# ZJU-Robotics-Lab/GEM

Hardware: AMD Instinct MI355X
Metric: fused points/sec into 600x600 grid; achieved HBM GB/s vs roofline (higher is better)
Workload: dtype f32

## Files before the change

gem_amd/build.py:

```python
from __future__ import annotations

import os
import shutil
import subprocess
from pathlib import Path

ROOT = Path(__file__).resolve().parent
CSRC = ROOT / "csrc"
LIBDIR = ROOT / "lib"
LIB = LIBDIR / "libgem_hip.so"

SOURCES = [CSRC / "gem_kernels.hip", CSRC / "gem_frame_lean.hip", CSRC / "gem_sort.hip", CSRC / "gem_capi.cpp", CSRC / "gem_capi_core.cpp", CSRC / "gem_capi_pipeline.cpp", CSRC / "gem_capi_comm.cpp",
           CSRC / "gem_clean.hip", CSRC / "gem_capi_clean.cpp", CSRC / "gem_local.hip", CSRC / "gem_capi_local.cpp",
           CSRC / "gem_voxel.hip", CSRC / "gem_capi_voxel.cpp", CSRC / "gem_global.hip", CSRC / "gem_capi_global.cpp",
           CSRC / "gem_compose.hip", CSRC / "gem_capi_compose.cpp", CSRC / "gem_costmap.hip", CSRC / "gem_capi_costmap.cpp",
           CSRC / "gem_octree.hip", CSRC / "gem_capi_octree.cpp", CSRC / "gem_depth.hip", CSRC / "gem_capi_depth.cpp",
           CSRC / "gem_history.hip", CSRC / "gem_capi_history.cpp",
           CSRC / "gem_footprint.hip", CSRC / "gem_capi_footprint.cpp", CSRC / "gem_inflate.hip", CSRC / "gem_capi_inflate.cpp",
           CSRC / "gem_mapgrid.hip", CSRC / "gem_capi_mapgrid.cpp", CSRC / "gem_critics.hip", CSRC / "gem_capi_critics.cpp",
           CSRC / "gem_trajgen.hip", CSRC / "gem_capi_trajgen.cpp", CSRC / "gem_navplan.hip", CSRC / "gem_capi_navplan.cpp",
           CSRC / "gem_frontier.hip", CSRC / "gem_capi_frontier.cpp", CSRC / "gem_obstacle.hip", CSRC / "gem_capi_obstacle.cpp",
           CSRC / "gem_voxlayer.hip", CSRC / "gem_capi_voxlayer.cpp"]
HEADERS = [CSRC / "gem_device.hpp", CSRC / "gem_kernels.hpp", CSRC / "gem_frame_lean.hpp", CSRC / "gem_frame_tile.hpp", CSRC / "gem_frame_sort.hpp", CSRC / "gem_wave.hpp", CSRC / "gem_compact.hpp", CSRC / "gem_transport.hpp", CSRC / "gem_hostcopy.hpp", CSRC / "gem_capi_internal.hpp", CSRC / "gem_plan.hpp", CSRC / "gem_clean.hpp", CSRC / "gem_local.hpp", CSRC / "gem_voxel.hpp", CSRC / "gem_global.hpp", CSRC / "gem_compose.hpp", CSRC / "gem_costmap.hpp", CSRC / "gem_lsd.hpp", CSRC / "gem_octree.hpp", CSRC / "gem_depth.hpp", CSRC / "gem_history.hpp", CSRC / "gem_footprint.hpp", CSRC / "gem_inflate.hpp", CSRC / "gem_mapgrid.hpp", CSRC / "gem_score_device.hpp", CSRC / "gem_critics.hpp", CSRC / "gem_trajgen.hpp", CSRC / "gem_sincos.hpp",
           CSRC / "gem_navplan.hpp", CSRC / "gem_navpath.hpp", CSRC / "gem_frontier.hpp", CSRC / "gem_costmap_host.hpp", CSRC / "gem_rounds.hpp", CSRC / "gem_tile_round.hpp", CSRC / "gem_obstacle.hpp", CSRC / "gem_voxlayer.hpp", ROOT.parent / "include" / "gem_hip_voxlayer.h", ROOT.parent / "include" / "gem_hip_frontier.h", ROOT.parent / "include" / "gem_hip_obstacle.h",
           ROOT.parent / "include" / "gem_hip_debug.h", ROOT.parent / "include" / "gem_hip.h", ROOT.parent / "include" / "gem_hip_history.h",
           ROOT.parent / "include" / "gem_hip_footprint.h", ROOT.parent / "include" / "gem_hip_inflate.h", ROOT.parent / "include" / "gem_hip_mapgrid.h",
           ROOT.parent / "include" / "gem_hip_critics.h", ROOT.parent / "include" / "gem_hip_trajgen.h", ROOT.parent / "include" / "gem_hip_navplan.h"]

FLAGS = [
    "--offload-arch=gfx950", "-O3", *(["-g"] if os.environ.get("GEM_DEBUG_BUILD") else []), "-std=c++17", "-ffp-contract=off", "-fPIC", "-shared",
    "-Wno-unused-value", "-Wno-unused-result",
    *os.environ.get("GEM_BUILD_DEFINES", "").split(),
]

SOURCE_FLAGS = {
    "gem_frame_lean.hip": ["-mllvm", "-amdgpu-kernarg-preload-count=14"],
}

# ... 99 lines not shown
```

gem_amd/csrc/gem_capi.cpp:

```cpp
#include "gem_capi_internal.hpp"
#include "gem_clean.hpp"
#include "gem_costmap.hpp"

namespace gemi {

int ensure_ray(gem_handle* h)
{
    if (h->ray.p) return GEM_OK;
    const int rc = ensure(h, h->ray, ((size_t)h->cells * 2 + 4) * sizeof(uint32_t));
    if (rc) return rc;
    GEM_HIP(h, hipMemsetAsync(static_cast<uint32_t*>(h->ray.p) + h->cells, 0, 4 * sizeof(uint32_t), h->stream));
    return GEM_OK;
}

static int queue_increment(gem_handle* h, float var_update)
{
    if (!(var_update >= 0.f)) h->floor_dirty = true;
    if (h->n_pending == kMaxPending) { int rc = flush_pending(h, false); if (rc) return rc; }
    h->pending[h->n_pending++] = var_update;
    return GEM_OK;
}

static int run_batch(gem_handle* h, int n_sweeps, const gem_frame_params* params, const float4* xyzi, const long long* offsets, const float* var_updates, bool caller_device)
{
// ... 186 lines not shown
    for (auto& ep : h->pool) { hipEventDestroy(ep.a); hipEventDestroy(ep.b); }
    local_free(h);
    global_free(h);
    costmap_free(h);
    history_free(h);
    octree_free(h);
    if (h->layers.elevation) hipFree(h->layers.elevation);
    if (h->d_counters) hipFree(h->d_counters);
    for (Arena* a : {&h->stage, &h->scratch, &h->dbg, &h->color, &h->ray, &h->sh_dev, &h->sh_recv_hv[0], &h->sh_recv_key[0], &h->sh_recv_rng[0],
                     &h->sh_recv_hv[1], &h->sh_recv_key[1], &h->sh_recv_rng[1], &h->sh_ranges, &h->published[0], &h->published[1],
                     &h->clean_cnt, &h->vox_state, &h->vox_hist, &h->vox_rec, &h->vox_tmp, &h->vox_out[0], &h->vox_out[1]}) if (a->p) hipFree(a->p);
    if (h->sh_host) hipHostFree(h->sh_host);
    if (h->form_seen) hipHostFree(h->form_seen);
    for (auto& b : h->pb) {
        for (Arena* a : {&b.rec, &b.srt, &b.seg, &b.flag, &b.gflag, &b.tables, &b.s_hv1, &b.s_hv2, &b.s_key1, &b.s_key2, &b.s_src1, &b.s_src2,
                         &b.s_cnt1, &b.s_cnt2, &b.s_misc, &b.s_ranges, &b.s_shard, &b.s_blkcnt}) if (a->p) hipFree(a->p);
        if (b.host_tables) hipHostFree(b.host_tables);
        if (b.tables_done) hipEventDestroy(b.tables_done);
        if (b.bin_done) hipEventDestroy(b.bin_done);
        if (b.fuse_done) hipEventDestroy(b.fuse_done);
    }
    if (h->copy_done) hipEventDestroy(h->copy_done);
    if (h->hstage) hipHostFree(h->hstage);
    for (auto& ev : h->ev_stage) if (ev) hipEventDestroy(ev);
    if (h->stage_read) hipEventDestroy(h->stage_read);
    for (auto& ev : h->ev_half) if (ev) hipEventDestroy(ev);
    if (h->switch_done) hipEventDestroy(h->switch_done);
    release_streams(h->device, h->streams);
    delete h;
}

// ... 4 lines not shown
    hipSetDevice(h->device);
    { const int rcd = settle(h); if (rcd) return rcd; }
    GEM_HIP(h, hipStreamSynchronize(h->stream));
    if (h->bin_stream) GEM_HIP(h, hipStreamSynchronize(h->bin_stream));
    if (h->bin_stream2) GEM_HIP(h, hipStreamSynchronize(h->bin_stream2));
    h->stream = hip_stream ? static_cast<hipStream_t>(hip_stream) : h->own_stream;
    return GEM_OK;
}

int gem_wait_event(gem_handle* h, void* hip_event)
{
    if (!h || !hip_event) return GEM_ERR_INVALID;
    std::lock_guard<std::mutex> lk(h->mu);
    hipSetDevice(h->device);
    hipEvent_t ev = static_cast<hipEvent_t>(hip_event);
    GEM_HIP(h, hipStreamWaitEvent(h->stream, ev, 0));
    if (h->bin_stream) GEM_HIP(h, hipStreamWaitEvent(h->bin_stream, ev, 0));
    if (h->bin_stream2) GEM_HIP(h, hipStreamWaitEvent(h->bin_stream2, ev, 0));
    h->main_reads_pb = true;
    return GEM_OK;
}

int gem_synchronize(gem_handle* h)
{
    ApiRange api_range(h, "gem_synchronize");
    if (!h) return GEM_ERR_INVALID;
    std::lock_guard<std::mutex> lk(h->mu);
    hipSetDevice(h->device);
    { const int rcd = settle(h); if (rcd) return rcd; }
    GEM_HIP(h, hipStreamSynchronize(h->stream));
// ... 237 lines not shown
    if (!h || n_sweeps <= 0 || !params || !offsets) return h ? fail(h, GEM_ERR_INVALID, "gem_add_batch_device: bad argument") : GEM_ERR_INVALID;
    std::lock_guard<std::mutex> lk(h->mu);
    hipSetDevice(h->device);
    { const int rcs = shard_finish_locked(h); if (rcs) return rcs; }
    for (int s = 0; s < n_sweeps; ++s) if (offsets[s + 1] < offsets[s]) return fail(h, GEM_ERR_INVALID, "gem_add_batch_device: offsets not monotone");
    return run_batch(h, n_sweeps, params, static_cast<const float4*>(d_xyzi), offsets, var_updates, true);
}

int gem_mapvar_update(gem_handle* h, float var_update)
{
    ApiRange api_range(h, "gem_mapvar_update");
    if (!h) return GEM_ERR_INVALID;
    std::lock_guard<std::mutex> lk(h->mu);
    hipSetDevice(h->device);
    { const int rcs = shard_finish_locked(h); if (rcs) return rcs; }
    return queue_increment(h, var_update);
}

static void* layer_ptr(gem_handle* h, int layer)
{
    switch (layer) {
    case GEM_LAYER_ELEVATION: return h->layers.elevation;
    case GEM_LAYER_VARIANCE:  return h->layers.variance;
    case GEM_LAYER_INTENSITY: return h->layers.intensity;
    case GEM_LAYER_TRAVER:    return h->layers.traver;
    case GEM_LAYER_LOWEST:    return h->layers.lowest;
    case GEM_LAYER_COLOR_R:   return h->layers.colorR;
    case GEM_LAYER_COLOR_G:   return h->layers.colorG;
    case GEM_LAYER_COLOR_B:   return h->layers.colorB;
    case GEM_LAYER_ROUGH:     return h->layers.rough;
// ... 248 lines not shown
    if (h->row0 != 0 || h->row1 != h->L) return fail(h, GEM_ERR_INVALID, "gem_raytracing: not available on a row-strip handle");
    int rc = flush_pending(h, false);
    if (rc) return rc;
    if ((rc = ensure_ray(h))) return rc;
    uint32_t* list = static_cast<uint32_t*>(h->ray.p);
    GEM_HIP(h, launch_raytracing(h->stream, h->layers, h->L, h->start[0], h->start[1], h->sensor_z, h->cfg.obstacle_threshold,
                                 h->row0, h->row1, list, list + h->cells, (int)(h->ray_calls++ & 1u), reinterpret_cast<float*>(list + h->cells + 4), h->ray_depth, h->ray_lanes));
    return GEM_OK;
}

int gem_set_timing(gem_handle* h, int enabled)
{
    if (!h) return GEM_ERR_INVALID;
    std::lock_guard<std::mutex> lk(h->mu);
    hipSetDevice(h->device);
    { const int rcd = settle(h); if (rcd) return rcd; }
    h->timing = enabled != 0;
    h->step_timed = h->timing && h->tp_x != nullptr && h->nranks > 1;
    return GEM_OK;
}

int gem_set_counting(gem_handle* h, int enabled)
{
    if (!h) return GEM_ERR_INVALID;
    std::lock_guard<std::mutex> lk(h->mu);
    hipSetDevice(h->device);
    { const int rcd = settle(h); if (rcd) return rcd; }
    h->counting = enabled != 0;
    return GEM_OK;
}

// ... 19 lines not shown
int gem_debug_set(gem_handle* h, const char* key, long long value)
{
    if (!h || !key) return GEM_ERR_INVALID;
    std::lock_guard<std::mutex> lk(h->mu);
    hipSetDevice(h->device);
    { const int rcd = settle(h); if (rcd) return rcd; }
    const std::string k(key);
    if (k == "fuse_variant")            { if (value < 10 || value > 12) return fail(h, GEM_ERR_INVALID, "fuse_variant: 10..12"); h->fuse_variant = (int)value; }
    else if (k == "tile_shift")         { if (value != 0 && value != 4 && value != 5) return fail(h, GEM_ERR_INVALID, "tile_shift: 0, 4 or 5"); h->ts = (int)value; }
    else if (k == "defer")              h->defer = value != 0;
    else if (k == "walk_always_wait")   h->walk_always_wait = value != 0;
    else if (k == "defer_walk")         { const int rcw = flush_walk(h); if (rcw) return rcw; h->defer_walk = value != 0; }
    else if (k == "dense_min")          { if (value < 0 || value > 0xffffffffll) return fail(h, GEM_ERR_INVALID, "dense_min: 0 .. 2^32 - 1"); h->dense_min = (unsigned)value; }
    else if (k == "dbg_sweep")          h->dbg_sweep = (int)value;
    else if (k == "dbg_frame")          h->dbg_frame = value != 0;
    else if (k == "frame_lean")         { if (value < 0 || value > 2) return fail(h, GEM_ERR_INVALID, "frame_lean: 0 (generic), 1 (lean) or 2 (the host picks)"); h->frame_lean = (int)value; }
    else if (k == "overlap")            h->overlap = value != 0;
    else if (k == "overlap_min_points") { if (value < 0) return fail(h, GEM_ERR_INVALID, "overlap_min_points: >= 0"); h->overlap_min_points = value; h->sort_overlap_min_points = value; }
    else if (k == "sort_path")          h->sort_path = value != 0;
    else if (k == "sort_min_points")    { if (value < 0) return fail(h, GEM_ERR_INVALID, "sort_min_points: >= 0"); h->sort_min_points = value; h->sort_min_points_batch = value; }
    else if (k == "walk_permute")       h->walk_permute = value != 0;
    else if (k == "trace")              h->trace = value != 0;
    else if (k == "stream_roles") {
        if (h->stream != h->own_stream) return fail(h, GEM_ERR_INVALID, "stream_roles: caller-provided stream in use");
        for (hipStream_t st : {h->own_stream, h->bin_stream, h->bin_stream2, h->tab_stream}) hipStreamSynchronize(st);
        const hipStream_t cur[4] = {h->own_stream, h->bin_stream, h->bin_stream2, h->tab_stream};
        const int d[4] = {(int)(value / 1000 % 10), (int)(value / 100 % 10), (int)(value / 10 % 10), (int)(value % 10)};
        bool seen[4] = {false, false, false, false};
        for (int i = 0; i < 4; ++i) { if (d[i] < 0 || d[i] > 3 || seen[d[i]]) return fail(h, GEM_ERR_INVALID, "stream_roles: not a permutation of 0123"); seen[d[i]] = true; }
        h->own_stream = cur[d[0]]; h->bin_stream = cur[d[1]]; h->bin_stream2 = cur[d[2]]; h->tab_stream = cur[d[3]];
// ... 36 lines not shown
    const std::string k(key);
    if (k == "arena_allocations") *out = h->arena_allocations;
    else if (k == "hstage_allocations") *out = h->hstage_allocations;
    else if (k == "copy_threads") *out = h->copy_threads;
    else if (k == "xfer_upload_memcpy_ns") *out = h->xfer_ns[0];
    else if (k == "xfer_upload_enqueue_ns") *out = h->xfer_ns[1];
    else if (k == "xfer_download_enqueue_ns") *out = h->xfer_ns[2];
    else if (k == "xfer_download_wait_ns") *out = h->xfer_ns[3];
    else if (k == "xfer_download_memcpy_ns") *out = h->xfer_ns[4];
    else if (k == "sort_fallbacks") *out = h->sort_fallbacks;
    else if (k == "compose_far_points") *out = h->compose.far_points;
    else if (k == "compose_sum_ns") *out = h->compose.sum_ns;
    else if (k == "walks_unwaited") *out = h->walks_unwaited;
    else if (k == "frame_lean_launches") *out = h->frame_lean_launches;
    else if (k == "frame_generic_launches") *out = h->frame_generic_launches;
    else if (k == "frame_form_seen") *out = h->form_seen ? (long long)*static_cast<volatile const uint32_t*>(h->form_seen) : 0;
    else if (k == "walks_left") *out = h->walks_left;
    else if (k == "history_cull") *out = h->history_cull ? 1 : 0;
    else if (k == "obstacle_direct") *out = h->obstacle_direct ? 1 : 0;
    else if (k == "nav_chunk") *out = h->nav_chunk;
    else if (k == "front_chunk") *out = h->front_chunk;
    else if (k == "history_blocks") *out = h->history.enabled ? cost_mark_blocks(h->history.len) : 0;
    else if (k == "history_blocks_culled") { hipSetDevice(h->device); return history_blocks_culled(h, out); }
    else if (k == "step_pending") *out = h->step.valid ? 1 : 0;
    else if (k == "step_exchange_bytes_out") *out = h->xbytes_out;
    else if (k == "step_exchange_bytes_in") *out = h->xbytes_in;
    else if (k == "gather_bytes_out") *out = h->gbytes_out;
    else if (k == "gather_bytes_in") *out = h->gbytes_in;
    else if (k.rfind("step_", 0) == 0) {
        int a = -1, b = -1;
// ... 44 lines not shown
```

gem_amd/csrc/gem_capi_core.cpp:

```cpp
#include "gem_capi_internal.hpp"

#include <cfloat>
#include <dlfcn.h>

namespace gemi {

thread_local std::string g_create_error;

namespace {
typedef int (*roctx_push_fn)(const char*);
typedef int (*roctx_pop_fn)();
std::once_flag g_roctx_once;
roctx_push_fn g_roctx_push = nullptr;
roctx_pop_fn g_roctx_pop = nullptr;
}

bool roctx_load()
{
    std::call_once(g_roctx_once, [] {
        for (const char* lib : {"librocprofiler-sdk-roctx.so", "librocprofiler-sdk-roctx.so.1", "libroctx64.so", "libroctx64.so.4"}) {
            void* so = dlopen(lib, RTLD_NOW | RTLD_GLOBAL);
            if (!so) continue;
            g_roctx_push = reinterpret_cast<roctx_push_fn>(dlsym(so, "roctxRangePushA"));
            g_roctx_pop = reinterpret_cast<roctx_pop_fn>(dlsym(so, "roctxRangePop"));
// ... 300 lines not shown
{
    hipEvent_t e = nullptr;
    hipEventCreate(&e);
    (void)h;
    return e;
}

void fold_events(gem_handle* h)
{
    for (auto& ep : h->events) {
        float ms = 0.f;
        if (hipEventSynchronize(ep.b) == hipSuccess && hipEventElapsedTime(&ms, ep.a, ep.b) == hipSuccess) {
            if (ep.kind == 0)      { h->stats.ms_bin += ms; h->stats.launches_bin++; }
            else if (ep.kind == 1) { h->stats.ms_fuse += ms; h->stats.launches_fuse++; }
            else if (ep.kind == 2) { h->stats.ms_frame += ms; h->stats.launches_frame++; }
            else if (ep.kind == 9) { h->stats.ms_walk += ms; h->stats.launches_walk++; }
            else                   { h->stats.ms_sort[ep.kind - 3] += ms; if (ep.kind == 3) h->stats.launches_sort++; }
        }
        else (void)hipGetLastError();
        h->pool.push_back(ep);
    }
    h->events.clear();
}

bool frame_launch_lean(gem_handle* h, bool fused_lean, bool bin_fast)
{
    const bool seen = h->form_seen && *static_cast<volatile const uint32_t*>(h->form_seen) != 0u;
    const bool lean = fused_lean && bin_fast && (h->frame_lean == 1 || (h->frame_lean == 2 && !seen));
    ++(lean ? h->frame_lean_launches : h->frame_generic_launches);
    return lean;
}

int flush_deferred(gem_handle* h)
{
    if (!h->deferred.valid) return GEM_OK;
    h->deferred.valid = false;
    h->main_reads_pb = true;
    if (h->dbg_frame) h->deferred.fa.dbg = nullptr;
    Timed t(h, 1);
    gem::BinArgs no_bin{};
    const bool lean = frame_launch_lean(h, h->deferred.lean_binned, true);
    GEM_HIP(h, launch_frame(h->stream, h->deferred.fa, no_bin, h->deferred.attr, lean, t.events()));
    return GEM_OK;
}

int flush_walk(gem_handle* h)
{
    if (!h->dwalk.valid) return GEM_OK;
    h->dwalk.valid = false;
    gem_handle::PassBuffers& pb = h->pb[h->dwalk.slot];
    if (!h->walk_always_wait && hipEventQuery(pb.bin_done) == hipSuccess) ++h->walks_unwaited;
    else { (void)hipGetLastError(); GEM_HIP(h, hipStreamWaitEvent(h->stream, pb.bin_done, 0)); }
    {
        Timed t(h, 9);
        GEM_HIP(h, h->dwalk.block_form ? launch_block_walk(h->stream, h->dwalk.wa, h->dwalk.attr, t.events()) : launch_walk(h->stream, h->dwalk.wa, h->dwalk.attr, t.events()));
    }
    GEM_HIP(h, hipEventRecord(pb.fuse_done, h->stream)); pb.fuse_recorded = true;
// ... 96 lines not shown
```

gem_amd/csrc/gem_capi_internal.hpp:

```cpp
#pragma once

#include "../../include/gem_hip.h"
#include "../../include/gem_hip_debug.h"
#include "gem_kernels.hpp"
#include "gem_plan.hpp"
#include "gem_hostcopy.hpp"
#include "gem_transport.hpp"

#include <hip/hip_runtime.h>
#include <rccl/rccl.h>

#include <chrono>
#include <cmath>
#include <cstdio>
#include <cstdlib>
#include <cstring>
#include <memory>
#include <mutex>
#include <string>
#include <vector>

using namespace gem;

namespace gem { struct CriticsArgs; struct FootSpec; struct CostGeom; }
// ... 45 lines not shown
        size_t host_cap = 0;
        hipEvent_t tables_done = nullptr;
        bool tables_recorded = false;
        std::vector<unsigned char> tab_key;
        int tab_src = 0;
        hipStream_t tab_upload_stream = nullptr;
        hipEvent_t bin_done = nullptr, fuse_done = nullptr;
        bool fuse_recorded = false;
        uint32_t epoch = 0;
    } pb[4];
    unsigned pass = 0, sort_pass = 0;
    uint32_t sort_epoch = 0;
    int sort_streams = 2;
    bool trace = false;
    int sort_ring = 3;
    struct Deferred { bool valid = false; FuseArgs fa{}; int ts = 0, attr = 0; bool lean_binned = false; } deferred;
    uint32_t* form_seen = nullptr;
    int  frame_lean = 2;
    long long frame_lean_launches = 0, frame_generic_launches = 0;
    struct DeferredWalk { bool valid = false; WalkArgs wa{}; bool block_form = false; int attr = 0; unsigned slot = 0; } dwalk;
    bool defer_walk = true;
    long long xbytes_out = 0, xbytes_in = 0, gbytes_out = 0, gbytes_in = 0;
    bool roctx = false;
    bool walk_always_wait = false;
    long long walks_unwaited = 0, walks_left = 0;
    bool defer = true;
    hipStream_t bin_stream = nullptr;
    hipStream_t bin_stream2 = nullptr;
    hipStream_t tab_stream = nullptr;
    hipEvent_t switch_done = nullptr;
    bool main_reads_pb = false;
// ... 279 lines not shown
    gem_handle* h; EventPair ep{};
    bool on;
    Timed(gem_handle* hh, int kind) : h(hh), on(hh->timing && kind >= 0)
    {
        if (!on) return;
        if (!h->pool.empty()) { ep = h->pool.back(); h->pool.pop_back(); }
        else { ep.a = get_event(h); ep.b = get_event(h); }
        ep.kind = kind;
    }
    LaunchEvents events() const { LaunchEvents e; if (on) { e.start = ep.a; e.stop = ep.b; } return e; }
    ~Timed() { if (on) h->events.push_back(ep); }
};

void fold_events(gem_handle* h);
int flush_deferred(gem_handle* h);
bool frame_launch_lean(gem_handle* h, bool fused_lean, bool bin_fast);
int flush_walk(gem_handle* h);
int flush_local(gem_handle* h);
int wait_gather(gem_handle* h);
void local_free(gem_handle* h);
int local_grid_count(gem_handle* h, uint32_t* n);
int local_export_to(gem_handle* h, void* dst, uint32_t n_grid, bool clear);
void compose_free(gem_handle* h);
int compose_check(gem_handle* h, const gem_compose_params* p, const char* what);
int compose_split(gem_handle* h, const gem_compose_params* p, bool want_road, bool want_obstacle, uint32_t tot[3], double* out_threshold);
void octree_free(gem_handle* h);
void global_free(gem_handle* h);
void history_free(gem_handle* h);
int history_check_room(gem_handle* h, long long n, const char* what);
int history_reserve(gem_handle* h, long long extra);
int history_append_device(gem_handle* h, const void* d_src, long long n);
// ... 94 lines not shown
```

gem_amd/csrc/gem_capi_pipeline.cpp:

```cpp
#include "gem_capi_internal.hpp"
#include "gem_clean.hpp"

namespace gemi {

static bool sort_bins_fit(int bins) { return sort_shape(bins, true, kSortChunkRecords).lds <= 160 * 1024; }
PlanEnv plan_env(const gem_handle* h)
{
    PlanEnv e{};
    e.L = h->L; e.ts = h->ts; e.sort_form = h->sort_form; e.sort_passes = h->sort_passes; e.sort_chunk = h->sort_chunk; e.sort_ring = h->sort_ring;
    e.sort_path = h->sort_path; e.track_lowest = h->track_lowest; e.sort_min_points = h->sort_min_points; e.sort_min_points_batch = h->sort_min_points_batch;
    return e;
}
SortGeometry sort_geometry(const gem_handle* h, int n_sweeps, bool block_form) { return sort_digits(h->L, h->sort_passes, n_sweeps, block_form, sort_bins_fit); }

static int stage_batch_tables(gem_handle* h, gem_handle::PassBuffers& pb, const TablesPlan& t, unsigned char** host = nullptr)
{
    if (t.total > pb.tables.cap) pb.tab_key.clear();
    const int rc = ensure(h, pb.tables, t.total);
    if (rc) return rc;
    if (t.total > pb.host_cap) {
        if (pb.tables_recorded) GEM_HIP(h, hipEventSynchronize(pb.tables_done));
        if (pb.host_tables) GEM_HIP(h, hipHostFree(pb.host_tables));
        pb.host_tables = nullptr; pb.host_cap = 0;
        GEM_HIP(h, hipHostMalloc(&pb.host_tables, t.total * 2, hipHostMallocDefault));
// ... 313 lines not shown
    std::vector<long long> cut_offsets;
    std::vector<int> orig0;
    if (plan.n_sweeps != in.n_sweeps) {
        const int ns = plan.n_sweeps;
        if (in.src == 0) cut_params.assign(ns, *in.params);
        cut_offsets.resize(ns + 1); orig0.resize(ns);
        for (int s = 0; s <= ns; ++s) cut_offsets[s] = std::min<long long>(in.n, (long long)s * kSweepPoints);
        for (int s = 0; s < ns; ++s) orig0[s] = (int)cut_offsets[s];
        in.n_sweeps = ns; in.params = in.src == 0 ? cut_params.data() : nullptr; in.offsets = cut_offsets.data(); in.var_updates = nullptr; in.sweep_orig0 = orig0.data();
    }
    const bool batched = in.n_sweeps > 1;
    const int U = kUnit, B = plan.B, bpad = plan.bpad;
    const bool dense = h->n_pending > 0 || h->floor_dirty || (batched && in.var_updates != nullptr);

    if (B == 0) {
        if (batched && in.var_updates)
            for (int s = 0; s < in.n_sweeps; ++s) {
                if (h->n_pending == kMaxPending) { int rc = flush_pending(h, true); if (rc) return rc; }
                h->pending[h->n_pending++] = in.var_updates[s];
            }
        return (h->n_pending || h->floor_dirty) ? flush_pending(h, true) : GEM_OK;
    }
    const int ts = plan.ts, tiles_per_row = plan.tiles_per_row, T = plan.T;
    h->T = T;
    if (fuse_lds_bytes(ts, h->fuse_variant, attr & 3) > 160 * 1024) return fail(h, GEM_ERR_INVALID, "fuse kernel geometry exceeds the LDS");

    bool overlap = h->overlap && in.n >= h->overlap_min_points && h->stream == h->own_stream && !h->counting && !h->dbg_on;
    const bool defer = h->defer && in.device_input && in.src == 0 && !batched && (attr & 3) == 0 && ts == 4 && !overlap &&
                       !h->counting && (!h->dbg_on || h->dbg_frame);
    if (!defer) { const int rcd = flush_deferred(h); if (rcd) return rcd; }
    gem_handle::PassBuffers& pb = h->pb[(overlap || defer) ? (h->pass++ & 1u) : 0u];
    hipStream_t sbin = overlap ? h->bin_stream : h->stream;
    int rc;
    if ((rc = switch_to_bin_streams(h, overlap))) return rc;
    if (overlap && pb.fuse_recorded) GEM_HIP(h, hipEventSynchronize(pb.fuse_done));
    static_assert(kSweepPoints <= (1ll << 22), "k_frame's record format");
    unsigned char* host = nullptr;
    if ((rc = ensure_tile_buffers(h, pb, plan, sbin, defer, &host))) return rc;
    if (pb.epoch >= kFlagEpochMax) {
        GEM_HIP(h, hipMemsetAsync(pb.flag.p, 0, pb.flag.cap, sbin));
        GEM_HIP(h, hipMemsetAsync(pb.gflag.p, 0, pb.gflag.cap, sbin));
        pb.epoch = 0;
    }
    ++pb.epoch;

    BinArgs ba{};
// ... 1 lines not shown
    const TablesPlan& tab = plan.tables;
    if (batched) {
        std::vector<int> unit0(in.n_sweeps + 1, 0);
        for (int s = 0; s < in.n_sweeps; ++s) unit0[s + 1] = unit0[s] + (int)sweep_units(in.offsets[s + 1] - in.offsets[s]);
        (void)fill_batch_tables(h, host, tab, in, unit0.data());
        GEM_HIP(h, hipMemcpyAsync(pb.tables.p, host, tab.total, hipMemcpyHostToDevice, sbin));
        GEM_HIP(h, hipEventRecord(pb.tables_done, sbin)); pb.tables_recorded = true;
        unsigned char* d = static_cast<unsigned char*>(pb.tables.p);
        ba.frames = reinterpret_cast<const FrameConst*>(d + tab.o_frames);
        ba.sweep_unit0 = reinterpret_cast<const int*>(d + tab.o_first0);
        ba.sweep_first = reinterpret_cast<const long long*>(d + tab.o_first);
        ba.sweep_orig0 = in.sweep_orig0 ? reinterpret_cast<const int*>(d + tab.o_orig) : nullptr;
        fa.sweep_unit0 = ba.sweep_unit0;
        fa.var_updates = in.var_updates ? reinterpret_cast<const float*>(d + tab.o_var) : nullptr;
    } else {
        fill_frame(h, in.src == 0 ? in.params : nullptr, ba.frame0);
    }
    ba.n_sweeps = in.n_sweeps; ba.n = in.n;
    ba.xyzi = in.xyzi; ba.rgb = in.rgb; ba.orig = in.orig;
    ba.f_index = in.f_index; ba.f_height = in.f_height; ba.f_var = in.f_var;
    ba.f_R = in.f_R; ba.f_G = in.f_G; ba.f_B = in.f_B; ba.f_I = in.f_I;
    ba.T = T; ba.tiles_per_row = tiles_per_row; ba.B = B; ba.Bpad = bpad;
    ba.tile_bits = 0; while ((1 << ba.tile_bits) < T) ++ba.tile_bits;
    ba.epoch = pb.epoch;
    ba.rec_words = (attr & 3) != 0 ? 4 : 3;
    ba.rec = static_cast<uint4*>(pb.rec.p); ba.seg = static_cast<uint16_t*>(pb.seg.p); ba.flag = static_cast<uint32_t*>(pb.flag.p); ba.gflag = static_cast<uint32_t*>(pb.gflag.p);
    ba.counters = h->counting ? h->d_counters : nullptr;
    ba.keep_sentinel = h->track_lowest ? 1 : 0;
    ba.srt_top = reinterpret_cast<uint32_t*>(static_cast<unsigned char*>(pb.srt.p) + pb.srt.cap - 16);

    fa.epoch = pb.epoch;
// ... 13 lines not shown
    fa.count_per_pass = orig0.empty() ? 0 : 1;
    fa.dbg = nullptr;
    fa.dbg_sweep = h->dbg_sweep;
    if (h->dbg_on) {
        const int nbin = (B + 3) / 4;
        if ((rc = ensure(h, h->dbg, (size_t)(T + nbin) * 16 * 8))) return rc;
        GEM_HIP(h, hipMemsetAsync(h->dbg.p, 0, (size_t)(T + nbin) * 16 * 8, h->stream));
        fa.dbg = static_cast<unsigned long long*>(h->dbg.p);
        if (h->dbg_frame) { ba.dbg = fa.dbg + (size_t)T * 16; h->dbg_rows = T + nbin; }
    }

    if (defer) {
        ba.bkt = static_cast<uint32_t*>(pb.bkt.p); ba.bcount = static_cast<uint32_t*>(pb.bcnt.p); ba.spill = static_cast<uint4*>(pb.spill.p);
        ba.ctl = static_cast<uint32_t*>(pb.fctl.p);
        fa.bkt = ba.bkt; fa.bcount = ba.bcount; fa.spill = ba.spill; fa.ctl = ba.ctl; fa.form_seen = h->form_seen;
        if (h->deferred.valid && h->deferred.attr != attr) { const int rcd = flush_deferred(h); if (rcd) return rcd; }
        const bool lean = frame_launch_lean(h, !h->deferred.valid || h->deferred.lean_binned, ba.frame0.fast_laser != 0 && !ba.rgb);
        ba.lean = lean ? 1 : 0;
        if (h->deferred.valid) { Timed t(h, 2); GEM_HIP(h, launch_frame(h->stream, h->deferred.fa, ba, attr, lean, t.events())); }
        else                   { Timed t(h, 0); GEM_HIP(h, launch_frame(h->stream, FuseArgs{}, ba, attr, lean, t.events())); }
        h->deferred.fa = fa; h->deferred.ts = ts; h->deferred.attr = attr; h->deferred.valid = true; h->deferred.lean_binned = lean;
        return pass_done(h, in.n);
    }
    if (h->counting) GEM_HIP(h, hipMemsetAsync(h->d_counters, 0, 2 * sizeof(unsigned long long), h->stream));
    { Timed t(h, 0); GEM_HIP(h, launch_bin(sbin, ba, in.src, ts, t.events())); }
    if (overlap) {
        GEM_HIP(h, hipEventRecord(pb.bin_done, sbin));
        GEM_HIP(h, hipStreamWaitEvent(h->stream, pb.bin_done, 0));
    }
    { Timed t(h, 1); GEM_HIP(h, launch_fuse(h->stream, fa, ts, attr, h->fuse_variant, t.events())); }
    if (overlap) { GEM_HIP(h, hipEventRecord(pb.fuse_done, h->stream)); pb.fuse_recorded = true; }
    return pass_done(h, in.n);
}

}

// ... 7 lines not shown
    int rc;
    if ((rc = ensure(h, h->stage, std::max({cloud_layout(max_points, true, true).bytes, stage_words_bytes(max_points, 9), depth_stage_bytes(max_points)})))) return rc;
    if ((rc = ensure(h, h->clean_cnt, clean_scratch_bytes(max_points)))) return rc;
    if ((rc = voxel_reserve(h, max_points))) return rc;
    const size_t one = stage_words_bytes(max_points, 7);
    size_t want = one < (16u << 20) ? 2 * one + 512 : 0;
    for (const size_t nine : {stage_words_bytes(max_points, 9), stage_words_bytes(h->cells, 9)}) if (nine <= (64u << 20)) want = std::max(want, nine);
    if (want) (void)host_stage(h, want);
    const bool sharded = h->tp_x && h->tile_strips;
    const PlanEnv env = plan_env(h);
    BoundPlan plan[kMaxBoundPlans];
    const int n_plans = bound_plans(env, max_points, max_sweeps, sharded ? h->nranks : 0, with_colours != 0, sort_bins_fit, plan);
    for (int i = 0; i < n_plans; ++i) {
        const BoundPlan& p = plan[i];
        for (int k = 0; p.kind == 1 && k < env.sort_ring; ++k) if ((rc = ensure_sort_buffers(h, h->pb[k], p.sort))) return rc;
        for (int k = 0; p.kind == 2 && k < 2; ++k) if ((rc = ensure_tile_buffers(h, h->pb[k], p.tile, h->stream, true))) return rc;
        if (sharded && p.kind == 1 && (rc = ensure_shard_tables(h, p.sort.blocks))) return rc;
    }
    if (sharded) {
        h->recv_bound = max_points;
        for (int q = 0; h->nranks > 1 && q < 2; ++q) if ((rc = ensure_recv(h, q, (size_t)max_points + 4 * h->nranks))) return rc;
    } else if (h->track_lowest && (rc = ensure_ray(h))) return rc;
    GEM_HIP(h, hipStreamSynchronize(h->stream));
    return GEM_OK;
}
```

gem_amd/csrc/gem_kernels.hpp:

```cpp
#pragma once

#include "gem_device.hpp"

namespace gem {

constexpr int kMaxPending = 4;
constexpr int kMaxRanks = 8;

constexpr int      kSegCountBits  = 7;
constexpr uint32_t kSegCountMask  = (1u << kSegCountBits) - 1u;
constexpr uint32_t kSegStartMask  = 63u;
constexpr uint32_t kFlagEpochMax  = 0xfffffff0u;

struct LayerPtrs {
    float *elevation, *variance, *intensity, *traver, *lowest;
    int   *colorR, *colorG, *colorB;
    float *rough, *slope;
};

constexpr int      kFrameBucket   = 768;
constexpr uint32_t kSpillFree     = 0xffffffffu;

struct BinArgs {
    FrameConst frame0;
// ... 173 lines not shown
constexpr int kSortChunkSmall = 1024;
inline int sort_chunk_for(long long n, int forced = 0)
{
    if (forced == kSortChunkRecords || forced == kSortChunkSmall) return forced;
    return n / kSortChunkRecords < 2 * 256 ? kSortChunkSmall : kSortChunkRecords;
}
constexpr int kSortMaxBins = 8000;

hipError_t launch_project(hipStream_t st, const FrameConst& fc, int first, int n, float* x, float* y, float* z, const int* orig,
                          int write_back, int* map_idx, float* var, float* xt, float* yt, float* zt);

hipError_t launch_bin(hipStream_t st, const BinArgs& a, int src, int ts, LaunchEvents ev);
hipError_t launch_fuse(hipStream_t st, const FuseArgs& a, int ts, int attr, int variant, LaunchEvents ev);
hipError_t launch_frame(hipStream_t st, const FuseArgs& fuse_prev, const BinArgs& bin_this, int attr, bool lean, LaunchEvents ev);
hipError_t launch_frame_lean(hipStream_t st, const FuseArgs& fuse_prev, const BinArgs& bin_this, int attr, unsigned blocks, LaunchEvents ev);
size_t     fuse_lds_bytes(int ts, int variant, int attr);
hipError_t launch_init(hipStream_t st, const LayerPtrs& m, int cells, int clear_lowest);
hipError_t launch_unpack_aos(hipStream_t st, const void* src, int n, int step, int ox, int oy, int oz, int oi, int orgb, float4* xyzi, uint32_t* rgb);
hipError_t launch_raytracing(hipStream_t st, const LayerPtrs& m, int L, int start0, int start1, float sensor_z, float obstacle_threshold,
                             int row0, int row1, uint32_t* list, uint32_t* counts, int parity, float* lowest_snapshot, int depth = 4, int lanes = 16);
hipError_t launch_clear_strip(hipStream_t st, const LayerPtrs& m, int L, int start, int count, int is_row);
hipError_t launch_dense_variance(hipStream_t st, float* variance, int cells, int n_pending, const float* pending,
                                 int apply_floor, float var_floor);
hipError_t launch_update_height(hipStream_t st, float* elevation, int cells, float dz);
hipError_t launch_map_feature(hipStream_t st, const float* elevation, float* traver, float* rough, float* slope,
                              int L, float res, int sx, int sy, int row0, int row1);
hipError_t launch_show(hipStream_t st, const LayerPtrs& m, int L, int sx, int sy, double map_length, double resolution, double px, double py,
                       uint32_t* block_count, float* visual, float* xyz, unsigned char* rgb, unsigned char* image, uint32_t* total);

struct ColorArgs {
// ... 17 lines not shown
```

Before: 25.23 billion.

## Pair two consecutive sweeps into a single fused frame kernel launch

```diff
diff --git a/gem_amd/build.py b/gem_amd/build.py
--- a/gem_amd/build.py
+++ b/gem_amd/build.py
@@ -10,7 +10,7 @@
 LIBDIR = ROOT / "lib"
 LIB = LIBDIR / "libgem_hip.so"
 
-SOURCES = [CSRC / "gem_kernels.hip", CSRC / "gem_frame_lean.hip", CSRC / "gem_sort.hip", CSRC / "gem_capi.cpp", CSRC / "gem_capi_core.cpp", CSRC / "gem_capi_pipeline.cpp", CSRC / "gem_capi_comm.cpp",
+SOURCES = [CSRC / "gem_kernels.hip", CSRC / "gem_frame_lean.hip", CSRC / "gem_frame_pair.hip", CSRC / "gem_sort.hip", CSRC / "gem_capi.cpp", CSRC / "gem_capi_core.cpp", CSRC / "gem_capi_pipeline.cpp", CSRC / "gem_capi_comm.cpp",
            CSRC / "gem_clean.hip", CSRC / "gem_capi_clean.cpp", CSRC / "gem_local.hip", CSRC / "gem_capi_local.cpp",
            CSRC / "gem_voxel.hip", CSRC / "gem_capi_voxel.cpp", CSRC / "gem_global.hip", CSRC / "gem_capi_global.cpp",
            CSRC / "gem_compose.hip", CSRC / "gem_capi_compose.cpp", CSRC / "gem_costmap.hip", CSRC / "gem_capi_costmap.cpp",
@@ -21,7 +21,7 @@
            CSRC / "gem_trajgen.hip", CSRC / "gem_capi_trajgen.cpp", CSRC / "gem_navplan.hip", CSRC / "gem_capi_navplan.cpp",
            CSRC / "gem_frontier.hip", CSRC / "gem_capi_frontier.cpp", CSRC / "gem_obstacle.hip", CSRC / "gem_capi_obstacle.cpp",
            CSRC / "gem_voxlayer.hip", CSRC / "gem_capi_voxlayer.cpp"]
-HEADERS = [CSRC / "gem_device.hpp", CSRC / "gem_kernels.hpp", CSRC / "gem_frame_lean.hpp", CSRC / "gem_frame_tile.hpp", CSRC / "gem_frame_sort.hpp", CSRC / "gem_wave.hpp", CSRC / "gem_compact.hpp", CSRC / "gem_transport.hpp", CSRC / "gem_hostcopy.hpp", CSRC / "gem_capi_internal.hpp", CSRC / "gem_plan.hpp", CSRC / "gem_clean.hpp", CSRC / "gem_local.hpp", CSRC / "gem_voxel.hpp", CSRC / "gem_global.hpp", CSRC / "gem_compose.hpp", CSRC / "gem_costmap.hpp", CSRC / "gem_lsd.hpp", CSRC / "gem_octree.hpp", CSRC / "gem_depth.hpp", CSRC / "gem_history.hpp", CSRC / "gem_footprint.hpp", CSRC / "gem_inflate.hpp", CSRC / "gem_mapgrid.hpp", CSRC / "gem_score_device.hpp", CSRC / "gem_critics.hpp", CSRC / "gem_trajgen.hpp", CSRC / "gem_sincos.hpp",
+HEADERS = [CSRC / "gem_device.hpp", CSRC / "gem_kernels.hpp", CSRC / "gem_frame_lean.hpp", CSRC / "gem_frame_pair.hpp", CSRC / "gem_frame_tile.hpp", CSRC / "gem_frame_sort.hpp", CSRC / "gem_wave.hpp", CSRC / "gem_compact.hpp", CSRC / "gem_transport.hpp", CSRC / "gem_hostcopy.hpp", CSRC / "gem_capi_internal.hpp", CSRC / "gem_plan.hpp", CSRC / "gem_clean.hpp", CSRC / "gem_local.hpp", CSRC / "gem_voxel.hpp", CSRC / "gem_global.hpp", CSRC / "gem_compose.hpp", CSRC / "gem_costmap.hpp", CSRC / "gem_lsd.hpp", CSRC / "gem_octree.hpp", CSRC / "gem_depth.hpp", CSRC / "gem_history.hpp", CSRC / "gem_footprint.hpp", CSRC / "gem_inflate.hpp", CSRC / "gem_mapgrid.hpp", CSRC / "gem_score_device.hpp", CSRC / "gem_critics.hpp", CSRC / "gem_trajgen.hpp", CSRC / "gem_sincos.hpp",
            CSRC / "gem_navplan.hpp", CSRC / "gem_navpath.hpp", CSRC / "gem_frontier.hpp", CSRC / "gem_costmap_host.hpp", CSRC / "gem_rounds.hpp", CSRC / "gem_tile_round.hpp", CSRC / "gem_obstacle.hpp", CSRC / "gem_voxlayer.hpp", ROOT.parent / "include" / "gem_hip_voxlayer.h", ROOT.parent / "include" / "gem_hip_frontier.h", ROOT.parent / "include" / "gem_hip_obstacle.h",
            ROOT.parent / "include" / "gem_hip_debug.h", ROOT.parent / "include" / "gem_hip.h", ROOT.parent / "include" / "gem_hip_history.h",
            ROOT.parent / "include" / "gem_hip_footprint.h", ROOT.parent / "include" / "gem_hip_inflate.h", ROOT.parent / "include" / "gem_hip_mapgrid.h",
diff --git a/gem_amd/csrc/gem_capi.cpp b/gem_amd/csrc/gem_capi.cpp
--- a/gem_amd/csrc/gem_capi.cpp
+++ b/gem_amd/csrc/gem_capi.cpp
@@ -224,7 +224,8 @@
     if (h->form_seen) hipHostFree(h->form_seen);
     for (auto& b : h->pb) {
         for (Arena* a : {&b.rec, &b.srt, &b.seg, &b.flag, &b.gflag, &b.tables, &b.s_hv1, &b.s_hv2, &b.s_key1, &b.s_key2, &b.s_src1, &b.s_src2,
-                         &b.s_cnt1, &b.s_cnt2, &b.s_misc, &b.s_ranges, &b.s_shard, &b.s_blkcnt}) if (a->p) hipFree(a->p);
+                         &b.s_cnt1, &b.s_cnt2, &b.s_misc, &b.s_ranges, &b.s_shard, &b.s_blkcnt,
+                         &b.bkt, &b.bcnt, &b.spill, &b.fctl}) if (a->p) hipFree(a->p);
         if (b.host_tables) hipHostFree(b.host_tables);
         if (b.tables_done) hipEventDestroy(b.tables_done);
         if (b.bin_done) hipEventDestroy(b.bin_done);
@@ -259,6 +260,7 @@
     std::lock_guard<std::mutex> lk(h->mu);
     hipSetDevice(h->device);
     hipEvent_t ev = static_cast<hipEvent_t>(hip_event);
+    { const int rcp = frame_unpair(h); if (rcp) return rcp; }
     GEM_HIP(h, hipStreamWaitEvent(h->stream, ev, 0));
     if (h->bin_stream) GEM_HIP(h, hipStreamWaitEvent(h->bin_stream, ev, 0));
     if (h->bin_stream2) GEM_HIP(h, hipStreamWaitEvent(h->bin_stream2, ev, 0));
@@ -526,6 +528,7 @@
     std::lock_guard<std::mutex> lk(h->mu);
     hipSetDevice(h->device);
     { const int rcs = shard_finish_locked(h); if (rcs) return rcs; }
+    { const int rcp = frame_unpair(h); if (rcp) return rcp; }
     return queue_increment(h, var_update);
 }
 
@@ -804,7 +807,7 @@
     if (!h) return GEM_ERR_INVALID;
     std::lock_guard<std::mutex> lk(h->mu);
     hipSetDevice(h->device);
-    { const int rcd = settle(h); if (rcd) return rcd; }
+    { int rcd = shard_finish_locked(h); if (!rcd) rcd = flush_walk(h); if (!rcd) rcd = wait_gather(h); if (rcd) return rcd; }
     h->timing = enabled != 0;
     h->step_timed = h->timing && h->tp_x != nullptr && h->nranks > 1;
     return GEM_OK;
@@ -854,6 +857,7 @@
     else if (k == "dense_min")          { if (value < 0 || value > 0xffffffffll) return fail(h, GEM_ERR_INVALID, "dense_min: 0 .. 2^32 - 1"); h->dense_min = (unsigned)value; }
     else if (k == "dbg_sweep")          h->dbg_sweep = (int)value;
     else if (k == "dbg_frame")          h->dbg_frame = value != 0;
+    else if (k == "frame_pair")         { if (value < 0 || value > 1) return fail(h, GEM_ERR_INVALID, "frame_pair: 0 (one launch per sweep) or 1 (two, for a stream nobody reads in between)"); h->frame_pair = value != 0; }
     else if (k == "frame_lean")         { if (value < 0 || value > 2) return fail(h, GEM_ERR_INVALID, "frame_lean: 0 (generic), 1 (lean) or 2 (the host picks)"); h->frame_lean = (int)value; }
     else if (k == "overlap")            h->overlap = value != 0;
     else if (k == "overlap_min_points") { if (value < 0) return fail(h, GEM_ERR_INVALID, "overlap_min_points: >= 0"); h->overlap_min_points = value; h->sort_overlap_min_points = value; }
@@ -920,6 +924,9 @@
     else if (k == "walks_unwaited") *out = h->walks_unwaited;
     else if (k == "frame_lean_launches") *out = h->frame_lean_launches;
     else if (k == "frame_generic_launches") *out = h->frame_generic_launches;
+    else if (k == "frame_pairs") *out = h->frame_pairs;
+    else if (k == "frame_held_flushed") *out = h->frame_held_flushed;
+    else if (k == "frame_pair") *out = h->frame_pair ? 1 : 0;
     else if (k == "frame_form_seen") *out = h->form_seen ? (long long)*static_cast<volatile const uint32_t*>(h->form_seen) : 0;
     else if (k == "walks_left") *out = h->walks_left;
     else if (k == "history_cull") *out = h->history_cull ? 1 : 0;
diff --git a/gem_amd/csrc/gem_capi_core.cpp b/gem_amd/csrc/gem_capi_core.cpp
--- a/gem_amd/csrc/gem_capi_core.cpp
+++ b/gem_amd/csrc/gem_capi_core.cpp
@@ -338,6 +338,7 @@
             if (ep.kind == 0)      { h->stats.ms_bin += ms; h->stats.launches_bin++; }
             else if (ep.kind == 1) { h->stats.ms_fuse += ms; h->stats.launches_fuse++; }
             else if (ep.kind == 2) { h->stats.ms_frame += ms; h->stats.launches_frame++; }
+            else if (ep.kind == 10) { h->stats.ms_frame += ms; h->stats.launches_frame += 2; }
             else if (ep.kind == 9) { h->stats.ms_walk += ms; h->stats.launches_walk++; }
             else                   { h->stats.ms_sort[ep.kind - 3] += ms; if (ep.kind == 3) h->stats.launches_sort++; }
         }
@@ -347,24 +348,73 @@
     h->events.clear();
 }
 
-bool frame_launch_lean(gem_handle* h, bool fused_lean, bool bin_fast)
+bool frame_would_lean(const gem_handle* h)
 {
     const bool seen = h->form_seen && *static_cast<volatile const uint32_t*>(h->form_seen) != 0u;
-    const bool lean = fused_lean && bin_fast && (h->frame_lean == 1 || (h->frame_lean == 2 && !seen));
-    ++(lean ? h->frame_lean_launches : h->frame_generic_launches);
+    return h->frame_lean == 1 || (h->frame_lean == 2 && !seen);
+}
+bool frame_launch_lean(gem_handle* h, bool fused_lean, bool bin_fast, int sweeps)
+{
+    const bool lean = fused_lean && bin_fast && frame_would_lean(h);
+    (lean ? h->frame_lean_launches : h->frame_generic_launches) += sweeps;
     return lean;
 }
 
+int frame_launch(gem_handle* h, gem_handle::FrameSweep* const* bins, int nb)
+{
+    const int nf = h->fstate.deferred;
+    if (nf + nb == 0) return GEM_OK;
+    bool fused_lean = true, bin_fast = true;
+    for (int i = 0; i < nf; ++i) fused_lean = fused_lean && h->deferred[i].lean_binned;
+    for (int i = 0; i < nb; ++i) bin_fast = bin_fast && bins[i]->ba.frame0.fast_laser != 0 && !bins[i]->ba.rgb;
+    const int attr = nb ? bins[0]->attr : h->deferred[0].attr;
+    const int most = nf > nb ? nf : nb;
+    const bool lean = frame_launch_lean(h, fused_lean, bin_fast, most);
+    for (int i = 0; i < nb; ++i) { bins[i]->ba.lean = lean ? 1 : 0; bins[i]->lean_binned = lean; }
+    const gem::FuseArgs no_fuse{};
+    const gem::BinArgs no_bin{};
+    if (most == 1) {
+        Timed t(h, nb == 0 ? 1 : nf == 0 ? 0 : 2);
+        GEM_HIP(h, launch_frame(h->stream, nf ? h->deferred[0].fa : no_fuse, nb ? bins[0]->ba : no_bin, attr, lean, t.events()));
+    } else if (lean && attr == 0) {
+        const gem::FuseArgs* fp[2] = {&h->deferred[0].fa, &h->deferred[1].fa};
+        const gem::BinArgs* bp[2] = {nb > 0 ? &bins[0]->ba : nullptr, nb > 1 ? &bins[1]->ba : nullptr};
+        Timed t(h, nb == 0 ? 1 : nf == 0 ? 0 : 10);
+        GEM_HIP(h, launch_frame_pair(h->stream, fp, nf, bp, nb, t.events()));
+        ++h->frame_pairs;
+    } else {
+        for (int i = 0; i < most; ++i) {
+            Timed t(h, i >= nb ? 1 : i >= nf ? 0 : 2);
+            GEM_HIP(h, launch_frame(h->stream, i < nf ? h->deferred[i].fa : no_fuse, i < nb ? bins[i]->ba : no_bin, attr, false, t.events()));
+        }
+    }
+    for (int i = 0; i < nb; ++i) h->deferred[i] = *bins[i];
+    h->fstate.deferred = nb;
+    return GEM_OK;
+}
+
 int flush_deferred(gem_handle* h)
 {
-    if (!h->deferred.valid) return GEM_OK;
-    h->deferred.valid = false;
+    if (!h->fstate.held && !h->fstate.deferred) { h->fstate.streak = 0; return GEM_OK; }
     h->main_reads_pb = true;
-    if (h->dbg_frame) h->deferred.fa.dbg = nullptr;
-    Timed t(h, 1);
-    gem::BinArgs no_bin{};
-    const bool lean = frame_launch_lean(h, h->deferred.lean_binned, true);
-    GEM_HIP(h, launch_frame(h->stream, h->deferred.fa, no_bin, h->deferred.attr, lean, t.events()));
+    gem::FramePairState s = h->fstate;
+    const gem::FramePairPlan plan = gem::frame_pair_step(s, gem::kFrameFlush);
+    if (plan.held_flushed) ++h->frame_held_flushed;
+    for (int k = 0; k < plan.n; ++k) {
+        for (int i = 0; h->dbg_frame && i < h->fstate.deferred; ++i) h->deferred[i].fa.dbg = nullptr;
+        gem_handle::FrameSweep* bins[1] = {&h->held};
+        const int rc = frame_launch(h, bins, plan.launch[k].bin);
+        h->fstate.held = false;
+        if (rc) { h->fstate = gem::FramePairState{}; return rc; }
+    }
+    h->fstate = s;
+    return GEM_OK;
+}
+
+int frame_unpair(gem_handle* h)
+{
+    if (h->fstate.held || h->fstate.deferred == 2) return flush_deferred(h);
+    h->fstate.streak = 0;
     return GEM_OK;
 }
 
diff --git a/gem_amd/csrc/gem_capi_internal.hpp b/gem_amd/csrc/gem_capi_internal.hpp
--- a/gem_amd/csrc/gem_capi_internal.hpp
+++ b/gem_amd/csrc/gem_capi_internal.hpp
@@ -3,6 +3,7 @@
 #include "../../include/gem_hip.h"
 #include "../../include/gem_hip_debug.h"
 #include "gem_kernels.hpp"
+#include "gem_frame_pair.hpp"
 #include "gem_plan.hpp"
 #include "gem_hostcopy.hpp"
 #include "gem_transport.hpp"
@@ -83,7 +84,11 @@
     int sort_streams = 2;
     bool trace = false;
     int sort_ring = 3;
-    struct Deferred { bool valid = false; FuseArgs fa{}; int ts = 0, attr = 0; bool lean_binned = false; } deferred;
+    struct FrameSweep { FuseArgs fa{}; BinArgs ba{}; int ts = 0, attr = 0, set = 0; bool lean_binned = false; };
+    FrameSweep deferred[2], held;
+    gem::FramePairState fstate;
+    bool frame_pair = true;
+    long long frame_pairs = 0, frame_held_flushed = 0;
     uint32_t* form_seen = nullptr;
     int  frame_lean = 2;
     long long frame_lean_launches = 0, frame_generic_launches = 0;
@@ -393,7 +398,10 @@
 
 void fold_events(gem_handle* h);
 int flush_deferred(gem_handle* h);
-bool frame_launch_lean(gem_handle* h, bool fused_lean, bool bin_fast);
+bool frame_would_lean(const gem_handle* h);
+bool frame_launch_lean(gem_handle* h, bool fused_lean, bool bin_fast, int sweeps = 1);
+int frame_launch(gem_handle* h, gem_handle::FrameSweep* const* bins, int nb);
+int frame_unpair(gem_handle* h);
 int flush_walk(gem_handle* h);
 int flush_local(gem_handle* h);
 int wait_gather(gem_handle* h);
diff --git a/gem_amd/csrc/gem_capi_pipeline.cpp b/gem_amd/csrc/gem_capi_pipeline.cpp
--- a/gem_amd/csrc/gem_capi_pipeline.cpp
+++ b/gem_amd/csrc/gem_capi_pipeline.cpp
@@ -351,6 +351,7 @@
     const bool dense = h->n_pending > 0 || h->floor_dirty || (batched && in.var_updates != nullptr);
 
     if (B == 0) {
+        { const int rcd = frame_unpair(h); if (rcd) return rcd; }
         if (batched && in.var_updates)
             for (int s = 0; s < in.n_sweeps; ++s) {
                 if (h->n_pending == kMaxPending) { int rc = flush_pending(h, true); if (rc) return rc; }
@@ -366,7 +367,20 @@
     const bool defer = h->defer && in.device_input && in.src == 0 && !batched && (attr & 3) == 0 && ts == 4 && !overlap &&
                        !h->counting && (!h->dbg_on || h->dbg_frame);
     if (!defer) { const int rcd = flush_deferred(h); if (rcd) return rcd; }
-    gem_handle::PassBuffers& pb = h->pb[(overlap || defer) ? (h->pass++ & 1u) : 0u];
+    gem::FrameConst frame0{};
+    if (!batched) fill_frame(h, in.src == 0 ? in.params : nullptr, frame0);
+    bool pairable = defer && h->frame_pair && attr == 0 && in.caller_device && h->stream == h->own_stream && in.n > 0 && !h->dbg_on && !h->counting &&
+                    frame0.fast_laser != 0 && !in.rgb && frame_would_lean(h);
+    for (int i = 0; pairable && i < h->fstate.deferred; ++i) pairable = h->deferred[i].lean_binned && h->deferred[i].attr == 0;
+    if (defer && !pairable) { const int rcd = frame_unpair(h); if (rcd) return rcd; }
+    unsigned set = 0;
+    if (defer) {
+        unsigned used = 0;
+        for (int i = 0; i < h->fstate.deferred; ++i) used |= 1u << h->deferred[i].set;
+        if (h->fstate.held) used |= 1u << h->held.set;
+        while (used & (1u << set)) ++set;
+    } else if (overlap) set = h->pass++ & 1u;
+    gem_handle::PassBuffers& pb = h->pb[set];
     hipStream_t sbin = overlap ? h->bin_stream : h->stream;
     int rc;
     if ((rc = switch_to_bin_streams(h, overlap))) return rc;
@@ -398,7 +412,7 @@
         fa.sweep_unit0 = ba.sweep_unit0;
         fa.var_updates = in.var_updates ? reinterpret_cast<const float*>(d + tab.o_var) : nullptr;
     } else {
-        fill_frame(h, in.src == 0 ? in.params : nullptr, ba.frame0);
+        ba.frame0 = frame0;
     }
     ba.n_sweeps = in.n_sweeps; ba.n = in.n;
     ba.xyzi = in.xyzi; ba.rgb = in.rgb; ba.orig = in.orig;
@@ -442,12 +456,20 @@
         ba.bkt = static_cast<uint32_t*>(pb.bkt.p); ba.bcount = static_cast<uint32_t*>(pb.bcnt.p); ba.spill = static_cast<uint4*>(pb.spill.p);
         ba.ctl = static_cast<uint32_t*>(pb.fctl.p);
         fa.bkt = ba.bkt; fa.bcount = ba.bcount; fa.spill = ba.spill; fa.ctl = ba.ctl; fa.form_seen = h->form_seen;
-        if (h->deferred.valid && h->deferred.attr != attr) { const int rcd = flush_deferred(h); if (rcd) return rcd; }
-        const bool lean = frame_launch_lean(h, !h->deferred.valid || h->deferred.lean_binned, ba.frame0.fast_laser != 0 && !ba.rgb);
-        ba.lean = lean ? 1 : 0;
-        if (h->deferred.valid) { Timed t(h, 2); GEM_HIP(h, launch_frame(h->stream, h->deferred.fa, ba, attr, lean, t.events())); }
-        else                   { Timed t(h, 0); GEM_HIP(h, launch_frame(h->stream, FuseArgs{}, ba, attr, lean, t.events())); }
-        h->deferred.fa = fa; h->deferred.ts = ts; h->deferred.attr = attr; h->deferred.valid = true; h->deferred.lean_binned = lean;
+        if (h->fstate.deferred && h->deferred[0].attr != attr) { const int rcd = flush_deferred(h); if (rcd) return rcd; }
+        gem_handle::FrameSweep sw;
+        sw.fa = fa; sw.ba = ba; sw.ts = ts; sw.attr = attr; sw.set = (int)set;
+        const gem::FramePairPlan fp = gem::frame_pair_step(h->fstate, pairable ? gem::kFramePairable : gem::kFrameSingle);
+        if (fp.hold) {
+            for (auto& other : h->pb) if (!other.bkt.p && (rc = ensure_tile_buffers(h, other, plan, h->stream, true))) { h->fstate.held = false; return rc; }
+            h->held = sw;
+            return pass_done(h, in.n);
+        }
+        const bool was_held = fp.launch[0].bin == 2;
+        h->fstate.deferred = fp.launch[0].fuse; h->fstate.held = false;
+        gem_handle::FrameSweep* bins[2] = {was_held ? &h->held : &sw, &sw};
+        if ((rc = frame_launch(h, bins, fp.launch[0].bin))) { h->fstate = gem::FramePairState{}; return rc; }
+        h->main_reads_pb = true;
         return pass_done(h, in.n);
     }
     if (h->counting) GEM_HIP(h, hipMemsetAsync(h->d_counters, 0, 2 * sizeof(unsigned long long), h->stream));
@@ -485,7 +507,8 @@
     for (int i = 0; i < n_plans; ++i) {
         const BoundPlan& p = plan[i];
         for (int k = 0; p.kind == 1 && k < env.sort_ring; ++k) if ((rc = ensure_sort_buffers(h, h->pb[k], p.sort))) return rc;
-        for (int k = 0; p.kind == 2 && k < 2; ++k) if ((rc = ensure_tile_buffers(h, h->pb[k], p.tile, h->stream, true))) return rc;
+        const int tile_sets = (p.kind == 2 && p.tile.ts == 4 && h->frame_pair && h->defer && !h->track_lowest) ? 4 : 2;
+        for (int k = 0; p.kind == 2 && k < tile_sets; ++k) if ((rc = ensure_tile_buffers(h, h->pb[k], p.tile, h->stream, true))) return rc;
         if (sharded && p.kind == 1 && (rc = ensure_shard_tables(h, p.sort.blocks))) return rc;
     }
     if (sharded) {
diff --git a/gem_amd/csrc/gem_frame_pair.hip b/gem_amd/csrc/gem_frame_pair.hip
--- /dev/null
+++ b/gem_amd/csrc/gem_frame_pair.hip
@@ -0,0 +1,54 @@
+#include "gem_frame_tile.hpp"
+#include "gem_frame_pair.hpp"
+
+#include <hip/hip_ext.h>
+
+namespace gem {
+
+template <int FLAGS>
+__global__ __launch_bounds__(256, kFrameLeanWG) void pair_k_frame(FramePairArgs pa)
+{
+    extern __shared__ __attribute__((aligned(16))) unsigned char lds_dyn[];
+    if ((int)blockIdx.x < pa.nf) {
+        frame_tile<FLAGS, false>(pa.s[0].t, (int)blockIdx.x, lds_dyn);
+        __syncthreads();
+        frame_tile<FLAGS, false>(pa.s[1].t, (int)blockIdx.x, lds_dyn);
+    } else {
+        const int block = (int)blockIdx.x - pa.nf;
+        if (block < pa.nbin[0]) {
+            bin_unit_lean(pa.s[0].b, (int)(block * 4 + (threadIdx.x >> 6)));
+            if (block == 0 && threadIdx.x == 0) pa.s[0].b.ctl[1] = 0u;
+        } else {
+            const int block1 = block - pa.nbin[0];
+            bin_unit_lean(pa.s[1].b, (int)(block1 * 4 + (threadIdx.x >> 6)));
+            if (block1 == 0 && threadIdx.x == 0) pa.s[1].b.ctl[1] = 0u;
+        }
+    }
+}
+
+#define GEM_LAUNCH(k, grid, block, lds, st, ev, ...)                                              \
+    do {                                                                                           \
+        if ((ev).start || (ev).stop) hipExtLaunchKernelGGL(k, grid, block, (uint32_t)(lds), st, (ev).start, (ev).stop, 0, __VA_ARGS__); \
+        else hipLaunchKernelGGL(k, grid, block, lds, st, __VA_ARGS__);                             \
+    } while (0)
+
+hipError_t launch_frame_pair(hipStream_t st, const FuseArgs* const* fuse, int nfuse, const BinArgs* const* bin, int nbin, LaunchEvents ev)
+{
+    if (nfuse < 0 || nfuse > 2 || nbin < 0 || nbin > 2 || nfuse + nbin == 0) return hipErrorInvalidValue;
+    FramePairArgs pa{};
+    const FuseArgs no_fuse{};
+    const BinArgs no_bin{};
+    for (int s = 0; s < 2; ++s) {
+        pa.s[s] = frame_lean_args(s < nfuse ? *fuse[s] : no_fuse, s < nbin ? *bin[s] : no_bin);
+        if (s >= nfuse) { pa.s[s].t.T = 0; pa.s[s].t.nf = 0; }
+        if (s >= nbin) pa.s[s].b.B = 0;
+        pa.nbin[s] = (pa.s[s].b.B + 3) / 4;
+        if (pa.s[s].t.nf > pa.nf) pa.nf = pa.s[s].t.nf;
+    }
+    const dim3 grid((unsigned)(pa.nf + pa.nbin[0] + pa.nbin[1])), block(256);
+    if (grid.x == 0) return hipSuccess;
+    GEM_LAUNCH((pair_k_frame<0>), grid, block, kFrameLds, st, ev, pa);
+    return hipGetLastError();
+}
+
+}
diff --git a/gem_amd/csrc/gem_frame_pair.hpp b/gem_amd/csrc/gem_frame_pair.hpp
--- /dev/null
+++ b/gem_amd/csrc/gem_frame_pair.hpp
@@ -0,0 +1,60 @@
+#pragma once
+
+#include "gem_frame_lean.hpp"
+
+namespace gem {
+
+struct FramePairState { int streak = 0; int deferred = 0; bool held = false; };
+
+enum FrameEvent {
+    kFramePairable = 0,
+    kFrameSingle   = 1,
+    kFrameFlush    = 2,
+};
+
+struct FramePairPlan {
+    int  n = 0;
+    struct Launch { int fuse, bin; } launch[3] = {};
+    bool hold = false;
+    bool held_flushed = false;
+    int  pairs = 0;
+};
+
+constexpr int kFramePairStreak = 2;
+
+inline FramePairPlan frame_pair_step(FramePairState& s, FrameEvent e)
+{
+    FramePairPlan p{};
+    auto launch = [&](int fuse, int bin) {
+        p.launch[p.n].fuse = fuse; p.launch[p.n].bin = bin; ++p.n;
+        if (fuse == 2 || bin == 2) ++p.pairs;
+        s.deferred = bin; s.held = false;
+    };
+    auto flush = [&]() {
+        if (s.held) { launch(s.deferred, 1); p.held_flushed = true; }
+        if (s.deferred) launch(s.deferred, 0);
+        s.streak = 0;
+    };
+    if (e == kFrameFlush) { flush(); return p; }
+    if (e == kFrameSingle) {
+        if (s.held || s.deferred == 2) flush();
+        s.streak = 0;
+        launch(s.deferred, 1);
+        return p;
+    }
+    if (s.held) { launch(s.deferred, 2); ++s.streak; return p; }
+    if (s.streak >= kFramePairStreak) { s.held = true; p.hold = true; ++s.streak; return p; }
+    launch(s.deferred, 1);
+    ++s.streak;
+    return p;
+}
+
+struct FramePairArgs {
+    int nf;
+    int nbin[2];
+    int pad_;
+    FrameLeanArgs s[2];
+};
+static_assert(sizeof(FramePairArgs) <= 16 + 2 * 352, "the pair kernel's arguments: a head and two lean blocks");
+
+}
diff --git a/gem_amd/csrc/gem_kernels.hpp b/gem_amd/csrc/gem_kernels.hpp
--- a/gem_amd/csrc/gem_kernels.hpp
+++ b/gem_amd/csrc/gem_kernels.hpp
@@ -211,6 +211,7 @@
 hipError_t launch_fuse(hipStream_t st, const FuseArgs& a, int ts, int attr, int variant, LaunchEvents ev);
 hipError_t launch_frame(hipStream_t st, const FuseArgs& fuse_prev, const BinArgs& bin_this, int attr, bool lean, LaunchEvents ev);
 hipError_t launch_frame_lean(hipStream_t st, const FuseArgs& fuse_prev, const BinArgs& bin_this, int attr, unsigned blocks, LaunchEvents ev);
+hipError_t launch_frame_pair(hipStream_t st, const FuseArgs* const* fuse, int nfuse, const BinArgs* const* bin, int nbin, LaunchEvents ev);
 size_t     fuse_lds_bytes(int ts, int variant, int attr);
 hipError_t launch_init(hipStream_t st, const LayerPtrs& m, int cells, int clear_lowest);
 hipError_t launch_unpack_aos(hipStream_t st, const void* src, int n, int step, int ox, int oy, int oz, int oi, int orgb, float4* xyzi, uint32_t* rgb);
```

After: 26.35 billion, median of 6. 1.04x the previous value.
